# sangyun884/HR-VITON

Measured on AMD Instinct MI355X. Metric: 1024x768 try-on images/sec (train_generator.py step: tocg+glue, G fwd/bwd, D fwd/bwd x2, VGG, Adam), higher is better.
Workload: dtype bf16; 1 GPU; BASELINE configs[3] (SURVEY 8d config #4, headline): train_generator.py 1024x768, 4 img/GPU, --fp16 (bf16 MFMA operands, fp32 accumulate), SPADE ng...; global_batch=4, height=1024, width=768, parallelism=dp1-allreduce, persistent_grid_cus=256, dist_backend=none (single process), world_size=1, rccl_ranks=0

## Files before the change

### hr-viton_amd/csrc/thin_conv.hip

```cpp
#include <stdlib.h>

#include "conv_params.h"

namespace hrv {

typedef unsigned u32x4 __attribute__((ext_vector_type(4)));
typedef float thin_f32x2 __attribute__((ext_vector_type(2)));
typedef __bf16 thin_bf16x2 __attribute__((ext_vector_type(2)));
__device__ __forceinline__ unsigned thin_pk_bf16(float a, float b) {
  const thin_f32x2 v = {a, b};
  return __builtin_bit_cast(unsigned, __builtin_convertvector(v, thin_bf16x2));
}

struct ThinParams {
  const void* src; int N, H, W, CK, cs, co; unsigned src_bytes;
  const float* w; int Cout, Cin, KH, KW; const float* sigma; float wscale; int transposed;
  int NC;
  const float* shift;
  const void* res; int res_cs, res_co, res_f32, res_mode;
  int act; float slope;
  void* out; int out_cs, out_co, out_f32;
  int pad, tiles, tx, ty;
  int full;
};

template <int TN, int KB, int KS, bool WIDE = false>
__global__ __launch_bounds__(256) void thin_conv_kernel(const ThinParams p) {
  constexpr int KH = KS == 9 ? 3 : 1, KW = KH;
  constexpr int PWD = 16 + KW - 1, PHT = 8 + KH - 1, PPIX = PWD * PHT;
  constexpr int SL = (2 * KB) | 1;
  constexpr int PS = SL * 16;
  constexpr int NP = 32 * TN;
  constexpr int WBYTES = KS * KB * NP * 32;
  constexpr int NI = (PPIX * SL + 63) / 64;
  constexpr int NQ = (NI + 3) / 4;
  extern __shared__ __attribute__((aligned(1024))) unsigned char smem[];
  unsigned char* const wl = smem;
  unsigned char* const patch = smem + ((WBYTES + 1023) & ~1023);
  float* const bias_l = reinterpret_cast<float*>(patch + NI * 1024);

  const int tid = threadIdx.x, lane = tid & 63;
  const int wave = __builtin_amdgcn_readfirstlane(tid >> 6);
  const int l31 = lane & 31, lh = lane >> 5;

  {
    const float inv = p.wscale / (p.sigma ? p.sigma[0] : 1.f);
    for (int idx = tid; idx < KS * KB * NP * 16; idx += 256) {
      const int kk = idx & 15;
      int t = idx >> 4;
      const int n = t % NP; t /= NP;
      const int kb = t % KB, tap = t / KB;
      const int k = kb * 16 + kk;
      float v = 0.f;
      if (k < p.CK && n < p.NC) {
        const int kh = tap / KW, kw = tap - kh * KW;
        v = p.transposed ? p.w[(((size_t)k * p.Cin + n) * KH + (KH - 1 - kh)) * KW + (KW - 1 - kw)]
                         : p.w[(((size_t)n * p.Cin + k) * KH + kh) * KW + kw];
        v *= inv;
      }
      const int half = (kk >> 3) ^ ((n >> 3) & 1);
      *reinterpret_cast<unsigned short*>(wl + ((tap * KB + kb) * NP + n) * 32 + half * 16 + (kk & 7) * 2) = f2bf(v);
    }
  }

  if constexpr (WIDE)
    for (int c = tid; c < NP; c += 256) bias_l[c] = p.shift ? p.shift[c] : 0.f;

  const rsrc_t rs = make_rsrc(p.src, p.src_bytes);
  int d_py[NQ], d_px[NQ];
  unsigned d_off[NQ];
  bool d_ok[NQ];
#pragma unroll
  for (int q = 0; q < NQ; ++q) {
    int j = wave + 4 * q;
    j = j < NI ? j : NI - 1;
    const int slot = 64 * j + lane;
    const int pix = slot / SL, s = slot - pix * SL;
    const int py = pix / PWD, px = pix - py * PWD;
    d_ok[q] = pix < PPIX && 8 * s < p.CK;
    d_py[q] = py; d_px[q] = px;
    d_off[q] = (unsigned)(((py * p.W + px) * p.cs + 8 * s) * 2);
  }
  auto tile_origin = [&](int t, int& n, int& y0, int& x0) {
    n = t / (p.tx * p.ty);
    const int r = t - n * (p.tx * p.ty);
    y0 = (r / p.tx) * 8; x0 = (r % p.tx) * 16;
  };
  auto issue = [&](int t) {
    int n, y0, x0;
    tile_origin(t, n, y0, x0);
    const unsigned base = (unsigned)((((n * p.H + y0 - p.pad) * p.W + x0 - p.pad) * p.cs + p.co) * 2);
#pragma unroll
    for (int q = 0; q < NQ; ++q) {
      int j = wave + 4 * q;
      j = j < NI ? j : NI - 1;
      const int y = y0 - p.pad + d_py[q], x = x0 - p.pad + d_px[q];
      const bool ok = d_ok[q] && (unsigned)y < (unsigned)p.H && (unsigned)x < (unsigned)p.W;
      dma16(rs, reinterpret_cast<float*>(patch + j * 1024), ok ? base + d_off[q] : 0xFFFFFFF0u, 0u);
    }
  };

  const unsigned char* const a_lane = patch + ((2 * wave + (l31 >> 4)) * PWD + (l31 & 15)) * PS + lh * 16;
  const unsigned char* const b_lane = wl + l31 * 32 + (lh ^ ((l31 >> 3) & 1)) * 16;

  int t = blockIdx.x;
  if (t < p.tiles) issue(t);
  __builtin_amdgcn_s_waitcnt(0 | (7 << 4) | (0 << 8));
  __syncthreads();
  for (; t < p.tiles; t += gridDim.x) {
    f32x16 acc[TN];
#pragma unroll
    for (int j = 0; j < TN; ++j)
#pragma unroll
      for (int e = 0; e < 16; ++e) acc[j][e] = 0.f;
#pragma unroll
    for (int tap = 0; tap < KS; ++tap) {
      const int kh = tap / KW, kw = tap - kh * KW;
#pragma unroll
      for (int kb = 0; kb < KB; ++kb) {
        const f32x4 a = *reinterpret_cast<const f32x4*>(a_lane + (kh * PWD + kw) * PS + kb * 32);
#pragma unroll
        for (int j = 0; j < TN; ++j) {
          const f32x4 b = *reinterpret_cast<const f32x4*>(b_lane + ((tap * KB + kb) * NP + j * 32) * 32);
          acc[j] = __builtin_amdgcn_mfma_f32_32x32x16_bf16(__builtin_bit_cast(bf16x8, b), __builtin_bit_cast(bf16x8, a), acc[j], 0, 0, 0);
        }
      }
    }
    __syncthreads();
    const int tn = t + gridDim.x;
    if (tn < p.tiles) issue(tn);

    {
      int n, y0, x0;
      tile_origin(t, n, y0, x0);
      const int y = y0 + 2 * wave + (l31 >> 4), x = x0 + (l31 & 15);
      if constexpr (WIDE) {
        if (y < p.H && x < p.W) {
          const float act_sl = p.act == HRV_ACT_NONE ? 1.f : (p.act == HRV_ACT_RELU ? 0.f : p.slope);
          unsigned short* const orow = reinterpret_cast<unsigned short*>(p.out) + (((size_t)n * p.H + y) * p.W + x) * p.out_cs + p.out_co + 8 * lh;
#pragma unroll
          for (int j = 0; j < TN; ++j)
#pragma unroll
            for (int h = 0; h < 2; ++h) {
              unsigned q[2][2];
#pragma unroll
              for (int gg = 0; gg < 2; ++gg) {
                const int g = 2 * h + gg;
                const f32x4 b4 = *reinterpret_cast<const f32x4*>(bias_l + j * 32 + 8 * g + 4 * lh);
                float v[4];
#pragma unroll
                for (int e = 0; e < 4; ++e) {
                  const float t = acc[j][4 * g + e] + b4[e];
                  v[e] = fmaxf(t, t * act_sl);
                }
                q[gg][0] = thin_pk_bf16(v[0], v[1]);
                q[gg][1] = thin_pk_bf16(v[2], v[3]);
              }
              const auto s0 = __builtin_amdgcn_permlane32_swap(q[0][0], q[1][0], false, false);
              const auto s1 = __builtin_amdgcn_permlane32_swap(q[0][1], q[1][1], false, false);
              u32x4 o;
              o[0] = s0[0]; o[1] = s1[0]; o[2] = s0[1]; o[3] = s1[1];
              *reinterpret_cast<u32x4*>(orow + j * 32 + 16 * h) = o;
            }
        }
      } else
      if (y < p.H && x < p.W) {
        const size_t pix = ((size_t)n * p.H + y) * p.W + x;
#pragma unroll
        for (int j = 0; j < TN; ++j)
#pragma unroll
          for (int g = 0; g < 4; ++g) {
            const int c0 = j * 32 + 8 * g + 4 * lh;
            if (c0 < p.NC) {
              f32x4 v;
#pragma unroll
              for (int e = 0; e < 4; ++e) v[e] = acc[j][4 * g + e] + ((p.shift && c0 + e < p.NC) ? p.shift[c0 + e] : 0.f);
              if (p.res) {
                const f32x4 r4 = ld4rt<true>(reinterpret_cast<const float*>(p.res), pix * p.res_cs + p.res_co + c0, p.res_f32);
#pragma unroll
                for (int e = 0; e < 4; ++e) v[e] = res_combine(v[e], r4[e], p.res_mode, p.slope);
              }
#pragma unroll
              for (int e = 0; e < 4; ++e) v[e] = (c0 + e < p.NC) ? apply_act(v[e], p.act, p.slope) : 0.f;
              st4rt<true>(reinterpret_cast<float*>(p.out), pix * p.out_cs + p.out_co + c0, v, p.out_f32);
            }
          }
      }
    }
    if (WIDE && p.full) {
      constexpr int NS = 2 * TN;
      static_assert(NS < 64, "vmcnt is six bits");
      __builtin_amdgcn_s_waitcnt((NS & 15) | (7 << 4) | (0 << 8) | ((NS >> 4) << 14));
    } else {
      __builtin_amdgcn_s_waitcnt(0 | (7 << 4) | (0 << 8));
    }
    __syncthreads();
  }
}

template <int TN, int KB, int KS, bool WIDE = false>
static int thin_launch(const ThinParams& p, hipStream_t st) {
  constexpr int KH = KS == 9 ? 3 : 1;
  constexpr int PPIX = (16 + KH - 1) * (8 + KH - 1), SL = (2 * KB) | 1;
  constexpr int WB = (KS * KB * 32 * TN * 32 + 1023) & ~1023;
  constexpr int PB = ((PPIX * SL + 63) / 64) * 1024;
  constexpr int LDS = WB + PB + (WIDE ? 32 * TN * 4 : 0);
  static_assert(LDS <= 160 * 1024, "thin conv: LDS");
  static bool attr_done_dev[HRV_MAX_DEVICES] = {false};
  bool& attr_done = attr_done_dev[current_device()];
  if (!attr_done) {
    if (hipFuncSetAttribute(reinterpret_cast<const void*>(&thin_conv_kernel<TN, KB, KS, WIDE>), hipFuncAttributeMaxDynamicSharedMemorySize, LDS) !=
        hipSuccess) {
      set_error("thin_conv: hipFuncSetAttribute(MaxDynamicSharedMemorySize=%d) failed", LDS);
      return HRV_ERR_LAUNCH;
    }
    attr_done = true;
  }
  const int n_cu = persistent_cus();
  int per_cu = (160 * 1024) / LDS;
  per_cu = per_cu < 1 ? 1 : (per_cu > 4 ? 4 : per_cu);
  int grid = n_cu * per_cu;
  if (grid > p.tiles) grid = p.tiles;
  hipLaunchKernelGGL((thin_conv_kernel<TN, KB, KS, WIDE>), dim3(grid), dim3(256), LDS, st, p);
  return check_launch("thin_conv_kernel");
}

}

using namespace hrv;

extern "C" int hrv_thin_conv_supported(int32_t KH, int32_t KW, int32_t src_channels, int32_t out_columns) {
  if (!((KH == 3 && KW == 3) || (KH == 1 && KW == 1))) return 0;
  const int kb = (src_channels + 15) / 16, tn = (out_columns + 31) / 32;
  const bool k9 = KH == 3;
  if (k9) return (tn == 1 && (kb == 5 || kb == 2 || kb == 1)) || (tn == 3 && kb == 2) || (tn == 2 && (kb == 1 || kb == 4));
  return (tn == 1 && kb == 5) || (tn == 3 && kb == 2) || (tn == 12 && kb == 5 && out_columns == 384);
}

extern "C" int hrv_thin_conv_bf16(const hrv_thin_conv_t* d, hrv_stream_t stream) {
  HRV_REQUIRE(d && d->src && d->w_oihw && d->out, "thin_conv: null pointer");
  HRV_REQUIRE(d->N > 0 && d->H > 0 && d->W > 0 && d->Cout > 0 && d->Cin > 0, "thin_conv: extent");
  HRV_REQUIRE(d->mode == 0 || d->mode == 1, "thin_conv: mode 0 (forward) or 1 (data gradient)");
  const int CK = d->mode == 0 ? d->Cin : d->Cout, NC = d->mode == 0 ? d->Cout : d->Cin;
  HRV_REQUIRE(d->src_channels >= CK && d->src_channels % 8 == 0 && d->src_cstride % 8 == 0 && d->src_coff % 8 == 0 &&
                  d->src_coff + d->src_channels <= d->src_cstride && ((uintptr_t)d->src & 15) == 0,
              "thin_conv: the bf16 source needs 8-channel granules");
  HRV_REQUIRE(hrv_thin_conv_supported(d->KH, d->KW, d->src_channels, NC), "thin_conv: shape (k=%d, %d source channels, %d columns) "
              "is not one of the instantiated thin layers", d->KH, d->src_channels, NC);
  HRV_REQUIRE(d->out_cstride % 4 == 0 && d->out_coff % 4 == 0 && d->out_coff + ((NC + 3) & ~3) <= d->out_cstride,
              "thin_conv: output slice (4-channel groups)");
  HRV_REQUIRE(!d->residual || (d->res_cstride % 4 == 0 && d->res_coff % 4 == 0), "thin_conv: residual slice");
  HRV_REQUIRE(d->res_mode == 0 || d->res_mode == 1, "thin_conv: res_mode");
  const int64_t bytes = (int64_t)d->N * d->H * d->W * d->src_cstride * 2;
  HRV_REQUIRE(bytes < (int64_t)0xFFFFFFF0, "thin_conv: source larger than the 32-bit buffer range");
  ThinParams p;
  p.src = d->src; p.N = d->N; p.H = d->H; p.W = d->W; p.CK = d->src_channels; p.cs = d->src_cstride; p.co = d->src_coff;
  p.src_bytes = (unsigned)bytes;
  p.w = d->w_oihw; p.Cout = d->Cout; p.Cin = d->Cin; p.KH = d->KH; p.KW = d->KW; p.sigma = d->sigma; p.wscale = d->wscale;
  p.transposed = d->mode;
  p.CK = CK;
  p.NC = NC;
  p.shift = d->shift;
  p.res = d->residual; p.res_cs = d->res_cstride; p.res_co = d->res_coff; p.res_f32 = d->res_bf16 ? 0 : 1; p.res_mode = d->res_mode;
  p.act = d->act; p.slope = d->act_slope;
  p.out = d->out; p.out_cs = d->out_cstride; p.out_co = d->out_coff; p.out_f32 = d->out_bf16 ? 0 : 1;
  p.pad = d->KH / 2;
  p.tx = (d->W + 15) / 16; p.ty = (d->H + 7) / 8; p.tiles = d->N * p.tx * p.ty;
  p.full = (d->W % 16 == 0 && d->H % 8 == 0) ? 1 : 0;
  hipStream_t st = (hipStream_t)stream;
  const int kb = (d->src_channels + 15) / 16, tn = (NC + 31) / 32;
  if (d->KH == 3) {
    if (tn == 1 && kb == 5) return thin_launch<1, 5, 9>(p, st);
    if (tn == 1 && kb == 2) return thin_launch<1, 2, 9>(p, st);
    if (tn == 1 && kb == 1) return thin_launch<1, 1, 9>(p, st);
    if (tn == 3 && kb == 2) return thin_launch<3, 2, 9>(p, st);
    if (tn == 2 && kb == 1) return thin_launch<2, 1, 9>(p, st);
    if (tn == 2 && kb == 4) return thin_launch<2, 4, 9>(p, st);
  } else {
    if (tn == 1 && kb == 5) return thin_launch<1, 5, 1>(p, st);
    if (tn == 3 && kb == 2) return thin_launch<3, 2, 1>(p, st);
    if (tn == 12 && kb == 5) {
      HRV_REQUIRE(d->act == HRV_ACT_NONE || d->act == HRV_ACT_RELU || (d->act == HRV_ACT_LRELU && d->act_slope >= 0.f && d->act_slope <= 1.f),
                  "thin_conv: the 384-column layer takes no activation, ReLU or LeakyReLU");
      HRV_REQUIRE(d->mode == 0 && !d->residual && d->out_bf16 && d->out_cstride % 8 == 0 && d->out_coff % 8 == 0 &&
                      ((uintptr_t)d->out & 15) == 0,
                  "thin_conv: the 384-column layer is forward-only, without residual, into a bf16 tensor with 8-channel granules");
      return thin_launch<12, 5, 1, true>(p, st);
    }
  }
  set_error("thin_conv: no instantiation");
  return HRV_ERR_ARG;
}
```

Before: 66.90 images/s.

## Add multi-stage patch ring and LDS-staged epilogue for thin 1x1 convs

Adds a new thin-conv kernel that keeps an NB-deep ring of input patches in LDS, so the DMA for upcoming tiles is issued while the current tile computes. A counted vmcnt wait replaces the full drain, and LDS fragment reads are software-pipelined ahead of the MFMAs. The epilogue stages the accumulators through LDS so that stores and residual loads are coalesced buffer ops. Only the two small 1x1 shapes (tn1/kb5, tn3/kb2) use the new path; 3x3 and the 384-column layer stay on the old kernel. The cost is more LDS per block, which can lower occupancy, plus more complex wait accounting.

```diff
diff --git a/hr-viton_amd/csrc/thin_conv.hip b/hr-viton_amd/csrc/thin_conv.hip
--- a/hr-viton_amd/csrc/thin_conv.hip
+++ b/hr-viton_amd/csrc/thin_conv.hip
@@ -1,31 +1,347 @@
 #include <stdlib.h>
 
+#include <type_traits>
+
 #include "conv_params.h"
 
 namespace hrv {
 
-typedef unsigned u32x4 __attribute__((ext_vector_type(4)));
 typedef float thin_f32x2 __attribute__((ext_vector_type(2)));
 typedef __bf16 thin_bf16x2 __attribute__((ext_vector_type(2)));
 __device__ __forceinline__ unsigned thin_pk_bf16(float a, float b) {
   const thin_f32x2 v = {a, b};
   return __builtin_bit_cast(unsigned, __builtin_convertvector(v, thin_bf16x2));
 }
+#if defined(__HIP_DEVICE_COMPILE__)
+__device__ __forceinline__ void thin_store8(u32x2 v, rsrc_t r, unsigned voff) { __builtin_amdgcn_raw_buffer_store_b64(v, r, (int)voff, 0, 0); }
+#else
+__device__ inline void thin_store8(u32x2, rsrc_t, unsigned) {}
+#endif
 
 struct ThinParams {
   const void* src; int N, H, W, CK, cs, co; unsigned src_bytes;
   const float* w; int Cout, Cin, KH, KW; const float* sigma; float wscale; int transposed;
   int NC;
   const float* shift;
-  const void* res; int res_cs, res_co, res_f32, res_mode;
+  const void* res; int res_cs, res_co, res_f32, res_mode; unsigned res_bytes;
   int act; float slope;
-  void* out; int out_cs, out_co, out_f32;
+  void* out; int out_cs, out_co, out_f32; unsigned out_bytes;
   int pad, tiles, tx, ty;
   int full;
 };
 
+template <int TN, int KB, int KS, int NB, int CJ>
+struct ThinGeom {
+  static_assert(NB >= 2 && NB <= 4, "ring of 2..4 patch stages");
+  static_assert(CJ == 1 || CJ == 2, "epilogue chunk: 32 or 64 columns");
+  static constexpr int KH = KS == 9 ? 3 : 1, KW = KH;
+  static constexpr int PWD = 16 + KW - 1, PHT = 8 + KH - 1, PPIX = PWD * PHT;
+  static constexpr int SL = (2 * KB) | 1;
+  static constexpr int PS = SL * 16;
+  static constexpr int NP = 32 * TN;
+  static constexpr int WBYTES = KS * KB * NP * 32;
+  static constexpr int WB = (WBYTES + 1023) & ~1023;
+  static constexpr int NI = (PPIX * SL + 63) / 64;
+  static constexpr int NQ = (NI + 3) / 4;
+  static constexpr int PB = NI * 1024;
+  static constexpr int BIAS = NP * 4;
+  static constexpr int ROWB = CJ * 128 + 16, STW = 32 * ROWB, ST = 4 * STW;
+  static constexpr int OFF_PATCH = WB, OFF_BIAS = WB + NB * PB, OFF_ST = OFF_BIAS + BIAS;
+  static constexpr int LDS = OFF_ST + ST;
+  static constexpr int NCH = (TN + CJ - 1) / CJ;
+  static constexpr int younger(int epi) { return (NB - 2) * NQ + (NB - 1) * epi > 63 ? 63 : (NB - 2) * NQ + (NB - 1) * epi; }
+};
+
+__device__ __forceinline__ void thin_vm_wait(int n) {
+  switch (n) {
+#define THIN_V(N) case N: __builtin_amdgcn_s_waitcnt(wait_vm(N)); break;
+#define THIN_V8(B) THIN_V(B) THIN_V(B + 1) THIN_V(B + 2) THIN_V(B + 3) THIN_V(B + 4) THIN_V(B + 5) THIN_V(B + 6) THIN_V(B + 7)
+    THIN_V8(0) THIN_V8(8) THIN_V8(16) THIN_V8(24) THIN_V8(32) THIN_V8(40) THIN_V8(48) THIN_V8(56)
+#undef THIN_V8
+#undef THIN_V
+    default: __builtin_amdgcn_s_waitcnt(wait_vm(0)); break;
+  }
+}
+
+#define THIN_RD16(DST, ADDR, OFF) asm volatile("ds_read_b128 %0, %1 offset:%2" : "=v"(DST) : "v"(ADDR), "n"(OFF) : "memory")
+#define THIN_WR16(ADDR, V, OFF) asm volatile("ds_write_b128 %0, %1 offset:%2" : : "v"(ADDR), "v"(V), "n"(OFF) : "memory")
+constexpr int thin_wait_lgkm(int n) { return 0x3F | (7 << 4) | (n << 8) | (3 << 14); }
+__device__ __forceinline__ void thin_lgkm_wait(int n) {
+  switch (n) {
+#define THIN_W(N) case N: __builtin_amdgcn_s_waitcnt(thin_wait_lgkm(N)); break;
+    THIN_W(0) THIN_W(1) THIN_W(2) THIN_W(3) THIN_W(4) THIN_W(5) THIN_W(6) THIN_W(7) THIN_W(8) THIN_W(9) THIN_W(10) THIN_W(11) THIN_W(12)
+    THIN_W(13) THIN_W(14)
+#undef THIN_W
+    default: __builtin_amdgcn_s_waitcnt(thin_wait_lgkm(0)); break;
+  }
+}
+
+template <int TN, int KB, int KS, int NB, int CJ>
+__global__ __launch_bounds__(256) void thin_conv_kernel(const ThinParams p) {
+  using G = ThinGeom<TN, KB, KS, NB, CJ>;
+  constexpr int KW = G::KW, PWD = G::PWD, PPIX = G::PPIX, SL = G::SL, PS = G::PS, NP = G::NP, NI = G::NI, NQ = G::NQ;
+  extern __shared__ __attribute__((aligned(1024))) unsigned char smem[];
+  unsigned char* const wl = smem;
+  unsigned char* const patch = smem + G::OFF_PATCH;
+  float* const bias_l = reinterpret_cast<float*>(smem + G::OFF_BIAS);
+  const unsigned lds0 = (unsigned)(size_t)(__attribute__((address_space(3))) unsigned char*)smem;
+
+  const int tid = threadIdx.x, lane = tid & 63;
+  const int wave = __builtin_amdgcn_readfirstlane(tid >> 6);
+  const int l31 = lane & 31, lh = lane >> 5;
+
+  {
+    const float inv = p.wscale / (p.sigma ? p.sigma[0] : 1.f);
+    for (int idx = tid; idx < KS * KB * NP * 16; idx += 256) {
+      const int kk = idx & 15;
+      int t = idx >> 4;
+      const int n = t % NP; t /= NP;
+      const int kb = t % KB, tap = t / KB;
+      const int k = kb * 16 + kk;
+      float v = 0.f;
+      if (k < p.CK && n < p.NC) {
+        const int kh = tap / KW, kw = tap - kh * KW;
+        v = p.transposed ? p.w[(((size_t)k * p.Cin + n) * G::KH + (G::KH - 1 - kh)) * KW + (KW - 1 - kw)]
+                         : p.w[(((size_t)n * p.Cin + k) * G::KH + kh) * KW + kw];
+        v *= inv;
+      }
+      const int half = (kk >> 3) ^ ((n >> 3) & 1);
+      *reinterpret_cast<unsigned short*>(wl + ((tap * KB + kb) * NP + n) * 32 + half * 16 + (kk & 7) * 2) = f2bf(v);
+    }
+    for (int c = tid; c < NP; c += 256) bias_l[c] = (p.shift && c < p.NC) ? p.shift[c] : 0.f;
+  }
+
+  const rsrc_t rs = make_rsrc(p.src, p.src_bytes);
+  int d_py[NQ], d_px[NQ];
+  unsigned d_off[NQ];
+  bool d_ok[NQ];
+#pragma unroll
+  for (int q = 0; q < NQ; ++q) {
+    int j = wave + 4 * q;
+    j = j < NI ? j : NI - 1;
+    const int slot = 64 * j + lane;
+    const int pix = slot / SL, s = slot - pix * SL;
+    const int py = pix / PWD, px = pix - py * PWD;
+    d_ok[q] = pix < PPIX && 8 * s < p.CK;
+    d_py[q] = py; d_px[q] = px;
+    d_off[q] = (unsigned)(((py * p.W + px) * p.cs + 8 * s) * 2);
+  }
+  auto tile_origin = [&](int t, int& n, int& y0, int& x0) {
+    n = t / (p.tx * p.ty);
+    const int r = t - n * (p.tx * p.ty);
+    y0 = (r / p.tx) * 8; x0 = (r % p.tx) * 16;
+  };
+  auto issue = [&](int t, int stage) {
+    int n, y0, x0;
+    tile_origin(t, n, y0, x0);
+    const unsigned base = (unsigned)((((n * p.H + y0 - p.pad) * p.W + x0 - p.pad) * p.cs + p.co) * 2);
+#pragma unroll
+    for (int q = 0; q < NQ; ++q) {
+      int j = wave + 4 * q;
+      j = j < NI ? j : NI - 1;
+      const int y = y0 - p.pad + d_py[q], x = x0 - p.pad + d_px[q];
+      const bool ok = d_ok[q] && (unsigned)y < (unsigned)p.H && (unsigned)x < (unsigned)p.W;
+      dma16(rs, reinterpret_cast<float*>(patch + stage * G::PB + j * 1024), ok ? base + d_off[q] : 0xFFFFFFF0u, 0u);
+    }
+  };
+
+  const unsigned a_lane = lds0 + G::OFF_PATCH + ((2 * wave + (l31 >> 4)) * PWD + (l31 & 15)) * PS + lh * 16;
+  const unsigned b_lane = lds0 + l31 * 32 + (lh ^ ((l31 >> 3) & 1)) * 16;
+  const unsigned bias_a = lds0 + G::OFF_BIAS;
+
+  int gc[G::NCH];
+  unsigned gi[G::NCH];
+#pragma unroll
+  for (int c = 0; c < G::NCH; ++c) {
+    const int jn = (TN - c * CJ) < CJ ? (TN - c * CJ) : CJ;
+    int g = ((p.NC + 3) >> 2) - c * CJ * 8;
+    g = g < 0 ? 0 : (g > jn * 8 ? jn * 8 : g);
+    gc[c] = g;
+    gi[c] = (65536u + (unsigned)g - 1u) / (unsigned)(g > 0 ? g : 1);
+  }
+  int epi = 0;
+#pragma unroll
+  for (int c = 0; c < G::NCH; ++c) epi += (gc[c] + 1) >> 1;
+  epi = p.res ? 2 * epi : epi;
+  const int vm_run = G::younger(epi);
+  const rsrc_t rs_out = make_rsrc(p.out, p.out_bytes);
+  const rsrc_t rs_res = make_rsrc(p.res, p.res ? p.res_bytes : 0u);
+  const bool has_res = p.res != nullptr;
+  const unsigned st_wave = lds0 + G::OFF_ST + wave * G::STW;
+  const unsigned st_lane = st_wave + l31 * G::ROWB + lh * 16;
+
+  {
+    int t = blockIdx.x;
+#pragma unroll
+    for (int q = 0; q < NB - 1; ++q, t += gridDim.x)
+      if (t < p.tiles) issue(t, q);
+  }
+  __builtin_amdgcn_s_waitcnt(wait_vm(0));
+  __builtin_amdgcn_s_barrier();
+  asm volatile("" ::: "memory");
+
+  int rb = 0;
+  for (int t = blockIdx.x; t < p.tiles; t += gridDim.x) {
+    const int t_new = t + (NB - 1) * (int)gridDim.x;
+    const bool more = t_new < p.tiles;
+    if (more) issue(t_new, rb == 0 ? NB - 1 : rb - 1);
+
+    f32x16 acc[TN];
+#pragma unroll
+    for (int j = 0; j < TN; ++j)
+#pragma unroll
+      for (int e = 0; e < 16; ++e) acc[j][e] = 0.f;
+    {
+      constexpr int S = KS * KB;
+      static_assert(TN + 1 <= 15, "lgkmcnt is a 4-bit counter");
+      constexpr int D0 = 12 / (TN + 1) < 1 ? 1 : 12 / (TN + 1);
+      constexpr int DEPTH = D0 < S - 1 ? D0 : (S - 1 < 1 ? 1 : S - 1);
+      const unsigned a_addr = a_lane + rb * G::PB;
+      f32x4 fr[DEPTH + 1][TN + 1];
+#pragma unroll
+      for (int s = -DEPTH; s < S; ++s) {
+        if (s + DEPTH < S) {
+          const int q = s + DEPTH, nx = q % (DEPTH + 1), tap = q / KB, kb = q - tap * KB, kh = tap / KW, kw = tap - kh * KW;
+          THIN_RD16(fr[nx][0], a_addr, (kh * PWD + kw) * PS + kb * 32);
+#pragma unroll
+          for (int j = 0; j < TN; ++j) {
+            const int full = ((tap * KB + kb) * NP + j * 32) * 32;
+            THIN_RD16(fr[nx][1 + j], b_lane + (unsigned)(full & ~32767), full & 32767);
+          }
+        }
+        if (s < 0) continue;
+        thin_lgkm_wait(((S - 1 - s) < DEPTH ? (S - 1 - s) : DEPTH) * (TN + 1));
+        __builtin_amdgcn_sched_barrier(0);
+        const int cur = s % (DEPTH + 1);
+#pragma unroll
+        for (int j = 0; j < TN; ++j)
+          acc[j] = __builtin_amdgcn_mfma_f32_32x32x16_bf16(__builtin_bit_cast(bf16x8, fr[cur][1 + j]), __builtin_bit_cast(bf16x8, fr[cur][0]),
+                                                           acc[j], 0, 0, 0);
+        __builtin_amdgcn_sched_barrier(0);
+      }
+    }
+
+    {
+      int n, y0, x0;
+      tile_origin(t, n, y0, x0);
+      {
+        const int yw = y0 + 2 * wave;
+        auto epilogue = [&](auto RT_, auto OF_) {
+        constexpr int RT = decltype(RT_)::value;
+        constexpr bool OF = decltype(OF_)::value != 0;
+        constexpr unsigned osz = OF ? 4u : 2u, rsz = RT == 1 ? 4u : 2u;
+#pragma unroll
+        for (int c = 0; c < G::NCH; ++c) {
+          const int jn = (TN - c * CJ) < CJ ? (TN - c * CJ) : CJ;
+#pragma unroll
+          for (int jj = 0; jj < jn; ++jj)
+#pragma unroll
+            for (int g = 0; g < 4; ++g) {
+              const int j = c * CJ + jj;
+              const f32x4 a4 = {acc[j][4 * g], acc[j][4 * g + 1], acc[j][4 * g + 2], acc[j][4 * g + 3]};
+              THIN_WR16(st_lane, a4, (jj * 8 + 2 * g) * 16);
+            }
+#pragma unroll
+          for (int m0 = 0; m0 < 4 * jn; m0 += 4) {
+            f32x4 a4[4], b4[4], r4[4];
+            unsigned pixo[4];
+            int c0[4];
+            bool ok[4];
+#pragma unroll
+            for (int mm = 0; mm < 4; ++mm) {
+              if ((m0 + mm) * 64 >= 32 * gc[c]) continue;
+              const unsigned i = (unsigned)((m0 + mm) * 64 + lane);
+              const bool in = i < 32u * (unsigned)gc[c];
+              const unsigned pix = in ? (i * gi[c]) >> 16 : 0u;
+              const unsigned grp = in ? i - pix * (unsigned)gc[c] : 0u;
+              const int y = yw + (int)(pix >> 4), x = x0 + (int)(pix & 15);
+              ok[mm] = in && y < p.H && x < p.W;
+              pixo[mm] = (unsigned)((n * p.H + y) * p.W + x);
+              c0[mm] = (c * CJ * 8 + (int)grp) * 4;
+              THIN_RD16(a4[mm], st_wave + pix * G::ROWB + grp * 16, 0);
+              THIN_RD16(b4[mm], bias_a + (unsigned)c0[mm] * 4, 0);
+            }
+            if constexpr (RT != 0) {
+#pragma unroll
+              for (int mm = 0; mm < 4; ++mm) {
+                if ((m0 + mm) * 64 >= 32 * gc[c]) continue;
+                const unsigned off = ok[mm] ? (pixo[mm] * (unsigned)p.res_cs + (unsigned)(p.res_co + c0[mm])) * rsz : 0xFFFFFFF0u;
+                if constexpr (RT == 1) {
+                  r4[mm] = load16(rs_res, off, 0);
+                } else {
+                  const u32x2 h = load8(rs_res, off, 0);
+                  const unsigned h0 = h[0], h1 = h[1];
+                  r4[mm][0] = __builtin_bit_cast(float, h0 << 16); r4[mm][1] = __builtin_bit_cast(float, h0 & 0xFFFF0000u);
+                  r4[mm][2] = __builtin_bit_cast(float, h1 << 16); r4[mm][3] = __builtin_bit_cast(float, h1 & 0xFFFF0000u);
+                }
+              }
+            }
+            __builtin_amdgcn_s_waitcnt(thin_wait_lgkm(0));
+            __builtin_amdgcn_sched_barrier(0);
+#pragma unroll
+            for (int mm = 0; mm < 4; ++mm) {
+              if ((m0 + mm) * 64 >= 32 * gc[c]) continue;
+              f32x4 v;
+#pragma unroll
+              for (int e = 0; e < 4; ++e) v[e] = a4[mm][e] + b4[mm][e];
+              if constexpr (RT != 0) {
+#pragma unroll
+                for (int e = 0; e < 4; ++e) v[e] = res_combine(v[e], r4[mm][e], p.res_mode, p.slope);
+              }
+#pragma unroll
+              for (int e = 0; e < 4; ++e) v[e] = (c0[mm] + e < p.NC) ? apply_act(v[e], p.act, p.slope) : 0.f;
+              const unsigned off = ok[mm] ? (pixo[mm] * (unsigned)p.out_cs + (unsigned)(p.out_co + c0[mm])) * osz : 0xFFFFFFF0u;
+              if constexpr (OF) {
+                store16(v, rs_out, off);
+              } else {
+                u32x2 h;
+                h[0] = thin_pk_bf16(v[0], v[1]);
+                h[1] = thin_pk_bf16(v[2], v[3]);
+                thin_store8(h, rs_out, off);
+              }
+            }
+          }
+        }
+        };
+        using I0 = std::integral_constant<int, 0>; using I1 = std::integral_constant<int, 1>; using I2 = std::integral_constant<int, 2>;
+        if (!has_res) { if (p.out_f32) epilogue(I0{}, I1{}); else epilogue(I0{}, I0{}); }
+        else if (p.res_f32) { if (p.out_f32) epilogue(I1{}, I1{}); else epilogue(I1{}, I0{}); }
+        else { if (p.out_f32) epilogue(I2{}, I1{}); else epilogue(I2{}, I0{}); }
+      }
+    }
+    thin_vm_wait((p.full && more) ? vm_run : 0);
+    __builtin_amdgcn_s_barrier();
+    asm volatile("" ::: "memory");
+    rb = rb == NB - 1 ? 0 : rb + 1;
+  }
+}
+
+template <int TN, int KB, int KS, int NB, int CJ>
+static int thin_launch(const ThinParams& p, hipStream_t st) {
+  using G = ThinGeom<TN, KB, KS, NB, CJ>;
+  constexpr int LDS = G::LDS;
+  static_assert(LDS <= 160 * 1024, "thin conv: LDS");
+  static bool attr_done_dev[HRV_MAX_DEVICES] = {false};
+  bool& attr_done = attr_done_dev[current_device()];
+  if (!attr_done) {
+    if (hipFuncSetAttribute(reinterpret_cast<const void*>(&thin_conv_kernel<TN, KB, KS, NB, CJ>), hipFuncAttributeMaxDynamicSharedMemorySize,
+                            LDS) != hipSuccess) {
+      set_error("thin_conv: hipFuncSetAttribute(MaxDynamicSharedMemorySize=%d) failed", LDS);
+      return HRV_ERR_LAUNCH;
+    }
+    attr_done = true;
+  }
+  const int n_cu = persistent_cus();
+  int per_cu = (160 * 1024) / LDS;
+  per_cu = per_cu < 1 ? 1 : (per_cu > 4 ? 4 : per_cu);
+  int grid = n_cu * per_cu;
+  if (grid > p.tiles) grid = p.tiles;
+  hipLaunchKernelGGL((thin_conv_kernel<TN, KB, KS, NB, CJ>), dim3(grid), dim3(256), LDS, st, p);
+  return check_launch("thin_conv_kernel");
+}
+
 template <int TN, int KB, int KS, bool WIDE = false>
-__global__ __launch_bounds__(256) void thin_conv_kernel(const ThinParams p) {
+__global__ __launch_bounds__(256) void thin_conv_v1_kernel(const ThinParams p) {
   constexpr int KH = KS == 9 ? 3 : 1, KW = KH;
   constexpr int PWD = 16 + KW - 1, PHT = 8 + KH - 1, PPIX = PWD * PHT;
   constexpr int SL = (2 * KB) | 1;
@@ -199,7 +515,7 @@
 }
 
 template <int TN, int KB, int KS, bool WIDE = false>
-static int thin_launch(const ThinParams& p, hipStream_t st) {
+static int thin_launch_v1(const ThinParams& p, hipStream_t st) {
   constexpr int KH = KS == 9 ? 3 : 1;
   constexpr int PPIX = (16 + KH - 1) * (8 + KH - 1), SL = (2 * KB) | 1;
   constexpr int WB = (KS * KB * 32 * TN * 32 + 1023) & ~1023;
@@ -209,7 +525,7 @@
   static bool attr_done_dev[HRV_MAX_DEVICES] = {false};
   bool& attr_done = attr_done_dev[current_device()];
   if (!attr_done) {
-    if (hipFuncSetAttribute(reinterpret_cast<const void*>(&thin_conv_kernel<TN, KB, KS, WIDE>), hipFuncAttributeMaxDynamicSharedMemorySize, LDS) !=
+    if (hipFuncSetAttribute(reinterpret_cast<const void*>(&thin_conv_v1_kernel<TN, KB, KS, WIDE>), hipFuncAttributeMaxDynamicSharedMemorySize, LDS) !=
         hipSuccess) {
       set_error("thin_conv: hipFuncSetAttribute(MaxDynamicSharedMemorySize=%d) failed", LDS);
       return HRV_ERR_LAUNCH;
@@ -221,7 +537,7 @@
   per_cu = per_cu < 1 ? 1 : (per_cu > 4 ? 4 : per_cu);
   int grid = n_cu * per_cu;
   if (grid > p.tiles) grid = p.tiles;
-  hipLaunchKernelGGL((thin_conv_kernel<TN, KB, KS, WIDE>), dim3(grid), dim3(256), LDS, st, p);
+  hipLaunchKernelGGL((thin_conv_v1_kernel<TN, KB, KS, WIDE>), dim3(grid), dim3(256), LDS, st, p);
   return check_launch("thin_conv_kernel");
 }
 
@@ -253,6 +569,10 @@
   HRV_REQUIRE(d->res_mode == 0 || d->res_mode == 1, "thin_conv: res_mode");
   const int64_t bytes = (int64_t)d->N * d->H * d->W * d->src_cstride * 2;
   HRV_REQUIRE(bytes < (int64_t)0xFFFFFFF0, "thin_conv: source larger than the 32-bit buffer range");
+  const int64_t out_bytes = (int64_t)d->N * d->H * d->W * d->out_cstride * (d->out_bf16 ? 2 : 4);
+  const int64_t res_bytes = d->residual ? (int64_t)d->N * d->H * d->W * d->res_cstride * (d->res_bf16 ? 2 : 4) : 0;
+  HRV_REQUIRE(out_bytes < (int64_t)0xFFFFFFF0 && res_bytes < (int64_t)0xFFFFFFF0, "thin_conv: output / residual larger than the 32-bit buffer range");
+  HRV_REQUIRE(!d->residual || d->res_coff + ((NC + 3) & ~3) <= d->res_cstride, "thin_conv: residual slice");
   ThinParams p;
   p.src = d->src; p.N = d->N; p.H = d->H; p.W = d->W; p.CK = d->src_channels; p.cs = d->src_cstride; p.co = d->src_coff;
   p.src_bytes = (unsigned)bytes;
@@ -262,30 +582,31 @@
   p.NC = NC;
   p.shift = d->shift;
   p.res = d->residual; p.res_cs = d->res_cstride; p.res_co = d->res_coff; p.res_f32 = d->res_bf16 ? 0 : 1; p.res_mode = d->res_mode;
+  p.res_bytes = (unsigned)res_bytes;
   p.act = d->act; p.slope = d->act_slope;
-  p.out = d->out; p.out_cs = d->out_cstride; p.out_co = d->out_coff; p.out_f32 = d->out_bf16 ? 0 : 1;
+  p.out = d->out; p.out_cs = d->out_cstride; p.out_co = d->out_coff; p.out_f32 = d->out_bf16 ? 0 : 1; p.out_bytes = (unsigned)out_bytes;
   p.pad = d->KH / 2;
   p.tx = (d->W + 15) / 16; p.ty = (d->H + 7) / 8; p.tiles = d->N * p.tx * p.ty;
   p.full = (d->W % 16 == 0 && d->H % 8 == 0) ? 1 : 0;
   hipStream_t st = (hipStream_t)stream;
   const int kb = (d->src_channels + 15) / 16, tn = (NC + 31) / 32;
   if (d->KH == 3) {
-    if (tn == 1 && kb == 5) return thin_launch<1, 5, 9>(p, st);
-    if (tn == 1 && kb == 2) return thin_launch<1, 2, 9>(p, st);
-    if (tn == 1 && kb == 1) return thin_launch<1, 1, 9>(p, st);
-    if (tn == 3 && kb == 2) return thin_launch<3, 2, 9>(p, st);
-    if (tn == 2 && kb == 1) return thin_launch<2, 1, 9>(p, st);
-    if (tn == 2 && kb == 4) return thin_launch<2, 4, 9>(p, st);
+    if (tn == 1 && kb == 5) return thin_launch_v1<1, 5, 9>(p, st);
+    if (tn == 1 && kb == 2) return thin_launch_v1<1, 2, 9>(p, st);
+    if (tn == 1 && kb == 1) return thin_launch_v1<1, 1, 9>(p, st);
+    if (tn == 3 && kb == 2) return thin_launch_v1<3, 2, 9>(p, st);
+    if (tn == 2 && kb == 1) return thin_launch_v1<2, 1, 9>(p, st);
+    if (tn == 2 && kb == 4) return thin_launch_v1<2, 4, 9>(p, st);
   } else {
-    if (tn == 1 && kb == 5) return thin_launch<1, 5, 1>(p, st);
-    if (tn == 3 && kb == 2) return thin_launch<3, 2, 1>(p, st);
+    if (tn == 1 && kb == 5) return thin_launch<1, 5, 1, 2, 1>(p, st);
+    if (tn == 3 && kb == 2) return thin_launch<3, 2, 1, 3, 2>(p, st);
     if (tn == 12 && kb == 5) {
       HRV_REQUIRE(d->act == HRV_ACT_NONE || d->act == HRV_ACT_RELU || (d->act == HRV_ACT_LRELU && d->act_slope >= 0.f && d->act_slope <= 1.f),
                   "thin_conv: the 384-column layer takes no activation, ReLU or LeakyReLU");
       HRV_REQUIRE(d->mode == 0 && !d->residual && d->out_bf16 && d->out_cstride % 8 == 0 && d->out_coff % 8 == 0 &&
                       ((uintptr_t)d->out & 15) == 0,
                   "thin_conv: the 384-column layer is forward-only, without residual, into a bf16 tensor with 8-channel granules");
-      return thin_launch<12, 5, 1, true>(p, st);
+      return thin_launch_v1<12, 5, 1, true>(p, st);
     }
   }
   set_error("thin_conv: no instantiation");
```

Result: no change. 66.69 images/s (-0.3%).
